# ecmwf-ifs/dwarf-p-cloudsc2-tl-ad

Hardware: AMD Instinct MI355X
Metric: CLOUDSC2 NL columns/sec (fp64, NLEV=137) (higher is better)
Workload: dtype f64

## Files before the change

### dwarf_p_cloudsc2_tl_ad_amd/csrc/cloudsc2_alloc.hip

```cpp

#include <array>
#include "cloudsc2_host.hpp"

using namespace cloudsc2;

namespace {

struct DevAlloc {
  size_t bytes = 0;
  size_t chunk = 0;
  std::vector<hipMemGenericAllocationHandle_t> handles;
};
size_t env_gib(const char* name, size_t dflt) {
  const char* e = getenv(name);
  return (e && atoll(e) > 0) ? (size_t)atoll(e) : dflt;
}
std::mutex g_alloc_mutex;
std::vector<std::pair<void*, DevAlloc>> g_allocs;

size_t search_budget(size_t bytes, size_t free_b) {
  double share = bytes > (env_gib("CLOUDSC2_PLACE_WHOLE_MAX_GB", 12) << 30) ? 0.85 : 0.6;
  if (const char* e = getenv("CLOUDSC2_PLACE_MAX_SHARE")) { const double v = atof(e); if (v > 0.0 && v <= 1.0) share = v; }
  size_t budget = (size_t)(share * (double)free_b);
  const size_t cap = env_gib("CLOUDSC2_PLACE_MAX_GB", 0) << 30;
// ... 243 lines not shown
    int ndev = 0;
    if (lws && hipGetDeviceCount(&ndev) == hipSuccess && ndev > 0) return atoi(lws) > ndev;
    return false;
  }();
  return shared;
}

int device_malloc_impl(void** out, size_t bytes, const ProbeFn* custom, PlacePolicy policy) {
  if (!out) return fail(CLOUDSC2_EINVAL, "cloudsc2_device_malloc: NULL result pointer");
  *out = nullptr;
  if (bytes == 0) return 0;
  std::lock_guard<std::mutex> place_lock(g_place_mutex);
  static const bool allow_custom = !(getenv("CLOUDSC2_PLACE_PROBE") && strcmp(getenv("CLOUDSC2_PLACE_PROBE"), "kernel") != 0);
  struct Scope { Scope(const ProbeFn* f) { g_custom_probe = f; } ~Scope() { g_custom_probe = nullptr; } } scope(allow_custom ? custom : nullptr);
  if (int rc = require_device()) return rc;
  (void)device_prepare();
  static const bool place_env_off = getenv("CLOUDSC2_PLACE") && atoi(getenv("CLOUDSC2_PLACE")) == 0;
  static const bool place_env_on = getenv("CLOUDSC2_PLACE") && atoi(getenv("CLOUDSC2_PLACE")) != 0;
  const bool place = policy == kPlaceSearch ? !place_env_off : (policy == kPlaceOnRequest ? place_env_on : false);
  static const char* mode = getenv("CLOUDSC2_PLACE_MODE");
  const bool chunks = mode && !strcmp(mode, "chunks");
  if (place && chunks && bytes >= (256u << 20)) {
    PlaceStats stc;
    return device_malloc_chunks(out, bytes, stc);
  }
  size_t ncand = 1, budget = 0;
  if (place && bytes >= (256u << 20) && !device_is_shared()) {
    const char* ec = getenv("CLOUDSC2_PLACE_CANDIDATES");
    const size_t span = env_gib("CLOUDSC2_PLACE_SPAN_GB", 96) << 30;
    const size_t want = (ec && atoi(ec) > 0) ? (size_t)atoi(ec) : std::min<size_t>(64, std::max<size_t>(12, (span + bytes - 1) / bytes));
    size_t free_b = 0, total_b = 0;
    HIP_TRY(hipMemGetInfo(&free_b, &total_b));
    budget = search_budget(bytes, free_b);
    ncand = std::max<size_t>(1, std::min(want, budget / bytes));
  }
  std::vector<void*> cand;
  auto grow = [&](size_t n) {
    for (size_t k = 0; k < n; ++k) {
      void* p = nullptr;
      if (hipMalloc(&p, bytes) != hipSuccess) { (void)hipGetLastError(); break; }
      cand.push_back(p);
    }
  };
  grow(ncand);
  if (cand.empty()) {
    (void)hipDeviceSynchronize();
    grow(1);
  }
  if (cand.empty()) { g_err = "cloudsc2_device_malloc: hipMalloc: out of memory"; return (int)hipErrorOutOfMemory; }
  size_t best = 0;
  PlaceStats st;
  if (cand.size() > 1) {
    static const char* pk = getenv("CLOUDSC2_PLACE_PROBE");
    const bool generic = !g_custom_probe;
    const bool use_write = generic && (!pk || strcmp(pk, "mixed") != 0), use_mixed = generic && (!pk || strcmp(pk, "write") != 0);
    std::vector<double> msw, msm;
    hipError_t e = hipSuccess;
    auto probe_from = [&](size_t first) {
      const size_t n = cand.size() - first;
      auto base = [&](size_t k) { return cand[first + k]; };
      std::vector<double> m, w;
      if (!generic) {
        for (size_t k = first; k < cand.size() && e == hipSuccess; ++k) e = hipMemsetAsync(cand[k], 0, bytes, nullptr);
        if (e == hipSuccess) e = probe_all(n, bytes, kProbeCustom, base, m);
      }
      if (use_mixed) e = probe_all(n, bytes, kProbeMixed, base, m);
      if (use_write && e == hipSuccess) e = probe_all(n, bytes, kProbeWrite, base, w);
      msm.insert(msm.end(), m.begin(), m.end());
      msw.insert(msw.end(), w.begin(), w.end());
    };
    probe_from(0);
    if (e == hipSuccess) {
      const std::vector<double>& v = msm.empty() ? msw : msm;
      const double lo = *std::min_element(v.begin(), v.end()), hi = *std::max_element(v.begin(), v.end());
      size_t free_b = 0, total_b = 0;
      if (hi < 1.04 * lo && hipMemGetInfo(&free_b, &total_b) == hipSuccess) {
        const size_t first = cand.size();
        const size_t held = first * bytes, left = budget > held ? budget - held : 0;
        grow(std::min(first, std::min((size_t)(0.7 * (double)free_b), left) / bytes));
        if (cand.size() > first) probe_from(first);
      }
    }
    if (e != hipSuccess) {
      for (auto p : cand) (void)hipFree(p);
      g_err = std::string("cloudsc2_device_malloc: placement probe: ") + hipGetErrorString(e);
      (void)hipGetLastError();
      return (int)e;
    }
    std::vector<double> score(cand.size(), 0.0);
    for (auto* v : {&msw, &msm})
      if (!v->empty()) {
        const double lo = *std::min_element(v->begin(), v->end());
        const double weight = (v == &msw && !msm.empty()) ? 0.2 : 1.0;
        for (size_t k = 0; k < cand.size(); ++k) score[k] += weight * (*v)[k] / lo;
      }
    for (size_t k = 0; k < cand.size(); ++k)
      if (score[k] < score[best]) best = k;
    if (getenv("CLOUDSC2_PLACE_VERBOSE")) {
      fprintf(stderr, "cloudsc2_device_malloc: %zu bytes, %zu candidates, probe ms %s/write:", bytes, cand.size(), generic ? "mixed" : "of the caller's sweep");
      for (size_t k = 0; k < cand.size(); ++k)
        fprintf(stderr, " %s%.4f/%.4f", k == best ? "*" : "", msm.empty() ? 0.0 : msm[k], msw.empty() ? 0.0 : msw[k]);
      fprintf(stderr, "\n");
    }
    std::vector<double> s = msm.empty() ? msw : msm;
    st.best_ms = s[best];
    std::sort(s.begin(), s.end());
    st.median_ms = s[s.size() / 2]; st.worst_ms = s.back();
    for (size_t k = 0; k < cand.size(); ++k)
      if (k != best) (void)hipFree(cand[k]);
    if (getenv("CLOUDSC2_PLACE_VERBOSE")) {
      std::vector<double> one(1, 0.0);
      if (!generic) (void)probe_all(1, bytes, kProbeCustom, [&](size_t) { return cand[best]; }, one);
      double m = 0.0, w = 0.0;
      (void)cloudsc2_device_probe(cand[best], bytes, kProbeMixed, 3, &m);
      (void)cloudsc2_device_probe(cand[best], bytes, kProbeWrite, 3, &w);
      fprintf(stderr, "cloudsc2_device_malloc: the chosen candidate after freeing the others: caller's sweep %.4f mixed %.4f write %.4f ms\n", one[0], m, w);
    }
  }
  st.candidates = (int)cand.size();
  (cand.size() > 1 ? g_searches : g_plain_allocs).fetch_add(1);
  if (getenv("CLOUDSC2_PLACE_VERBOSE") && cand.size() == 1)
    fprintf(stderr, "cloudsc2_device_malloc: %zu bytes, 1 candidate (plain hipMalloc%s)\n", bytes,
            policy == kPlaceSearch ? "" : policy == kPlaceOnRequest ? "; host-array driver workspace: searched only with CLOUDSC2_PLACE=1" : "; staging");
  DevAlloc a;
  a.bytes = bytes;
  std::lock_guard<std::mutex> lock(g_alloc_mutex);
  g_allocs.emplace_back(cand[best], a);
  g_last_place = st;
  *out = cand[best];
  return 0;
}

int device_free_impl(void* p) {
  if (!p) return 0;
  DevAlloc a;
  {
    std::lock_guard<std::mutex> lock(g_alloc_mutex);
    auto it = std::find_if(g_allocs.begin(), g_allocs.end(), [&](const std::pair<void*, DevAlloc>& x) { return x.first == p; });
    if (it == g_allocs.end()) return fail(CLOUDSC2_EINVAL, "cloudsc2_device_free: not a pointer returned by cloudsc2_device_malloc");
    a = it->second;
    g_allocs.erase(it);
  }
  if (a.chunk) {
    HIP_TRY(hipDeviceSynchronize());
    for (size_t k = 0; k < a.handles.size(); ++k) (void)hipMemUnmap((char*)p + k * a.chunk, a.chunk);
    for (auto x : a.handles) (void)hipMemRelease(x);
    (void)hipMemAddressFree(p, a.bytes);
    return 0;
  }
  HIP_TRY(hipFree(p));
  return 0;
}

}

extern "C" {
int cloudsc2_device_malloc(void** ptr, size_t bytes) { return device_malloc_impl(ptr, bytes); }
int cloudsc2_device_free(void* ptr) { return device_free_impl(ptr); }
int cloudsc2_device_probe(void* ptr, size_t bytes, int kind, int rounds, double* ms) {
  if (!ptr || !ms || rounds < 1 || rounds > 64 || (kind != 0 && kind != 1)) return fail(CLOUDSC2_EINVAL, "cloudsc2_device_probe: bad argument");
  if (int rc = require_device()) return rc;
  const long long nblocks = kind == 0 ? (long long)(bytes / (size_t)kProbeBlockBytes) : (long long)(bytes / (size_t)((kMixIn + kMixOut) * kMixBlockElems * 8));
  if (nblocks < 1 || nblocks > 0x7fffffffLL) return fail(CLOUDSC2_EINVAL, "cloudsc2_device_probe: buffer too small or too large");
  hipEvent_t ea = nullptr, eb = nullptr;
  hipError_t e = hipEventCreate(&ea);
  if (e == hipSuccess) e = hipEventCreate(&eb);
  std::vector<float> t;
  for (int r = 0; r <= rounds && e == hipSuccess; ++r) {
    (void)hipEventRecord(ea, nullptr);
    launch_probe(ptr, bytes, kind);
    (void)hipEventRecord(eb, nullptr);
    e = hipEventSynchronize(eb);
    float f = 0;
    if (e == hipSuccess) e = hipEventElapsedTime(&f, ea, eb);
    if (r > 0) t.push_back(f);
  }
  if (ea) (void)hipEventDestroy(ea);
  if (eb) (void)hipEventDestroy(eb);
  if (e != hipSuccess) { g_err = std::string("cloudsc2_device_probe: ") + hipGetErrorString(e); (void)hipGetLastError(); return (int)e; }
  std::sort(t.begin(), t.end());
  *ms = t[t.size() / 2];
  return 0;
}
void cloudsc2_device_malloc_counts(long long* searched, long long* plain) {
  if (searched) *searched = g_searches.load();
  if (plain) *plain = g_plain_allocs.load();
}
void cloudsc2_device_malloc_info(int* candidates, double* best_ms, double* median_ms, double* worst_ms) {
  std::lock_guard<std::mutex> lock(g_alloc_mutex);
  if (candidates) *candidates = g_last_place.candidates;
  if (best_ms) *best_ms = g_last_place.best_ms;
  if (median_ms) *median_ms = g_last_place.median_ms;
  if (worst_ms) *worst_ms = g_last_place.worst_ms;
}
}
```

### dwarf_p_cloudsc2_tl_ad_amd/csrc/cloudsc2_driver.hip

```cpp

#include <thread>
#include "cloudsc2_host.hpp"

using namespace cloudsc2;

namespace {


__global__ void __launch_bounds__(256)
scale_planes_kernel(real_t* dst, long long dst_stride, const real_t* src, long long src_stride, long long plane, long long nblocks,
                    real_t factor) {
  long long i = (long long)blockIdx.x * blockDim.x + threadIdx.x;
  if (i >= plane * nblocks) return;
  long long ibl = i / plane, r = i - ibl * plane;
  dst[ibl * dst_stride + r] = src[ibl * src_stride + r] * factor;
}

__global__ void __launch_bounds__(256)
reblock_kernel(const real_t* __restrict__ src, int np_src, long long stride_src, real_t* __restrict__ dst, int np_dst,
               long long stride_dst, long long nrows, long long ncopy, long long nzero) {
  const long long total = nrows * nzero;
  for (long long e = (long long)blockIdx.x * blockDim.x + threadIdx.x; e < total; e += (long long)gridDim.x * blockDim.x) {
    const long long row = e / nzero, g = e - row * nzero;
    const long long bd = g / np_dst, jd = g - bd * np_dst;
    real_t v = 0;
    if (g < ncopy) {
      const long long bs = g / np_src, js = g - bs * np_src;
      v = src[bs * stride_src + row * np_src + js];
    }
    dst[bd * stride_dst + row * np_dst + jd] = v;
  }
}

constexpr size_t kAlignReals = 256 / sizeof(real_t);
size_t r32(size_t n) { return (n + kAlignReals - 1) & ~(kAlignReals - 1); }
constexpr size_t kF64 = sizeof(double) / sizeof(real_t);

struct Arena {
  real_t* base = nullptr;
  size_t cap = 0, used = 0;
  int device = -1;

  int reserve(size_t nreals, const ProbeFn* probe = nullptr, PlacePolicy policy = kPlaceSearch) {
    int dev = 0;
    HIP_TRY(hipGetDevice(&dev));
    if (base && (cap < nreals || dev != device)) { (void)device_free_impl(base); base = nullptr; cap = 0; }
    if (!base) {
      int rc = device_malloc_impl((void**)&base, nreals * sizeof(real_t), probe, policy);
      if (rc) { base = nullptr; return rc; }
      cap = nreals;
      device = dev;
    }
    used = 0;
    return 0;
  }
  real_t* take(size_t n) {
    n = r32(n);
    real_t* p = base + used;
    used += n;
    return p;
  }
  double* take_f64(size_t n) { return (double*)take(n * (sizeof(double) / sizeof(real_t))); }
  void release() {
    if (base) (void)device_free_impl(base);
    base = nullptr; cap = 0; used = 0;
  }
};
Arena g_arena;
std::mutex g_arena_mutex;

struct DevState {
  real_t *pt, *pq, *b_cml, *b_loc, *pap, *paph, *plu, *plude, *pmfu, *pmfd, *pa, *pclv, *psupsat, *pcovptot;
  real_t *pfplsl, *pfplsn, *pfhpsl, *pfhpsn, *qsat;
  long long S, H;
  long long nblocks;
};

size_t state_out_reals(long long ncols_pad, int nlev) {
  size_t s = (size_t)ncols_pad * nlev, h = (size_t)ncols_pad * (nlev + 1);
  return 3 * r32(s) + 4 * r32(h) + r32(8 * s);
}
size_t state_in_reals(long long ncols_pad, int nlev) {
  size_t s = (size_t)ncols_pad * nlev, h = (size_t)ncols_pad * (nlev + 1);
  return 8 * r32(s) + r32(h) + r32(8 * s) + r32(5 * s);
}
size_t state_reals(long long ncols_pad, int nlev) { return state_in_reals(ncols_pad, nlev) + state_out_reals(ncols_pad, nlev); }

void state_take(Arena& a, DevState& d, long long ncols_pad, int nproma, int nlev) {
  Arena& ain = a;
  Arena& aout = a;
  size_t s = (size_t)ncols_pad * nlev, h = (size_t)ncols_pad * (nlev + 1);
  d.S = (long long)nproma * nlev;
  d.H = (long long)nproma * (nlev + 1);
  d.nblocks = ncols_pad / nproma;
  d.pt = ain.take(s); d.pq = ain.take(s); d.pap = ain.take(s); d.plu = ain.take(s); d.plude = ain.take(s);
  d.pmfu = ain.take(s); d.pmfd = ain.take(s); d.psupsat = ain.take(s);
  d.paph = ain.take(h); d.b_cml = ain.take(8 * s); d.pclv = ain.take(5 * s);
  d.pa = aout.take(s); d.pcovptot = aout.take(s); d.qsat = aout.take(s);
  d.pfplsl = aout.take(h); d.pfplsn = aout.take(h); d.pfhpsl = aout.take(h); d.pfhpsn = aout.take(h);
  d.b_loc = aout.take(8 * s);
}

struct HostState {
  const real_t *pt, *pq, *b_cml; real_t* b_loc;
  const real_t *pap, *paph, *plu, *plude, *pmfu, *pmfd; real_t* pa; const real_t *pclv, *psupsat;
  real_t *pcovptot, *pfplsl, *pfplsn, *pfhpsl, *pfhpsn;
};

int copy_planes(real_t* dst, const real_t* src, long long plane_off, long long plane, long long block_stride, long long nblocks,
                hipMemcpyKind kind, hipStream_t st) {
  if (nblocks <= 0) return 0;
  HIP_TRY(hipMemcpy2DAsync(dst + plane_off, block_stride * sizeof(real_t), src + plane_off, block_stride * sizeof(real_t),
                           plane * sizeof(real_t), (size_t)nblocks, kind, st));
  return 0;
}

int upload(const HostState& h, const DevState& d, long long ncols_pad, int nlev, hipStream_t st) {
  size_t s = (size_t)ncols_pad * nlev * sizeof(real_t), hh = (size_t)ncols_pad * (nlev + 1) * sizeof(real_t);
  const long long P = d.S;
  HIP_TRY(hipMemcpyAsync(d.pt, h.pt, s, hipMemcpyHostToDevice, st));
  HIP_TRY(hipMemcpyAsync(d.pq, h.pq, s, hipMemcpyHostToDevice, st));
  HIP_TRY(hipMemcpyAsync(d.pap, h.pap, s, hipMemcpyHostToDevice, st));
  HIP_TRY(hipMemcpyAsync(d.paph, h.paph, hh, hipMemcpyHostToDevice, st));
  HIP_TRY(hipMemcpyAsync(d.plu, h.plu, s, hipMemcpyHostToDevice, st));
  HIP_TRY(hipMemcpyAsync(d.plude, h.plude, s, hipMemcpyHostToDevice, st));
  HIP_TRY(hipMemcpyAsync(d.pmfu, h.pmfu, s, hipMemcpyHostToDevice, st));
  HIP_TRY(hipMemcpyAsync(d.pmfd, h.pmfd, s, hipMemcpyHostToDevice, st));
  HIP_TRY(hipMemcpyAsync(d.psupsat, h.psupsat, s, hipMemcpyHostToDevice, st));
  int rc;
  for (int p : {0, 2, 3, 4})
    if ((rc = copy_planes(d.b_cml, h.b_cml, p * P, P, 8 * P, d.nblocks, hipMemcpyHostToDevice, st))) return rc;
  for (int p : {0, 1})
    if ((rc = copy_planes(d.pclv, h.pclv, p * P, P, 5 * P, d.nblocks, hipMemcpyHostToDevice, st))) return rc;
  return 0;
}

int download_active2(real_t* hdst, long long hstride, const real_t* dsrc, long long dstride, long long nlevx, int nproma,
                     long long ngptot, hipStream_t st) {
  const long long nfull = ngptot / nproma, icend = ngptot - nfull * nproma;
  const long long plane = (long long)nproma * nlevx;
  if (nfull > 0) {
    if (hstride == plane && dstride == plane) {
      HIP_TRY(hipMemcpyAsync(hdst, dsrc, (size_t)nfull * plane * sizeof(real_t), hipMemcpyDeviceToHost, st));
    } else {
      HIP_TRY(hipMemcpy2DAsync(hdst, hstride * sizeof(real_t), dsrc, dstride * sizeof(real_t), plane * sizeof(real_t), (size_t)nfull,
                               hipMemcpyDeviceToHost, st));
    }
  }
  if (icend > 0) {
    HIP_TRY(hipMemcpy2DAsync(hdst + nfull * hstride, (size_t)nproma * sizeof(real_t), dsrc + nfull * dstride, (size_t)nproma * sizeof(real_t),
                             (size_t)icend * sizeof(real_t), (size_t)nlevx, hipMemcpyDeviceToHost, st));
  }
  return 0;
}
int download_active(real_t* hdst, const real_t* dsrc, long long plane_off, long long nlevx, long long block_stride, int nproma,
                    long long ngptot, hipStream_t st) {
  return download_active2(hdst + plane_off, block_stride, dsrc + plane_off, block_stride, nlevx, nproma, ngptot, st);
}

int download(const HostState& h, const DevState& d, long long ncols_pad, int nlev, hipStream_t st, int nproma, long long ngptot) {
  const long long P = d.S, PH = d.H;
  int rc;
  for (int p : {0, 2, 3, 4})
    if ((rc = download_active(h.b_loc, d.b_loc, p * P, nlev, 8 * P, nproma, ngptot, st))) return rc;
  if ((rc = copy_planes(h.b_loc, d.b_loc, 7 * P, P, 8 * P, d.nblocks, hipMemcpyDeviceToHost, st))) return rc;
  if ((rc = download_active(h.pa, d.pa, 0, nlev, P, nproma, ngptot, st))) return rc;
  HIP_TRY(hipMemcpyAsync(h.pcovptot, d.pcovptot, (size_t)ncols_pad * nlev * sizeof(real_t), hipMemcpyDeviceToHost, st));
  if ((rc = download_active(h.pfplsl, d.pfplsl, 0, nlev + 1, PH, nproma, ngptot, st))) return rc;
  if ((rc = download_active(h.pfplsn, d.pfplsn, 0, nlev + 1, PH, nproma, ngptot, st))) return rc;
  if ((rc = download_active(h.pfhpsl, d.pfhpsl, 0, nlev + 1, PH, nproma, ngptot, st))) return rc;
  if ((rc = download_active(h.pfhpsn, d.pfhpsn, 0, nlev + 1, PH, nproma, ngptot, st))) return rc;
  return 0;
}

cloudsc2_field fld(real_t* p, long long stride) { cloudsc2_field f; f.ptr = p; f.block_stride = stride; return f; }

void traj_blocks(const DevState& d, int nproma, int nlev, bool with_qsat, cloudsc2_inputs& in, cloudsc2_outputs& out) {
  const long long S = d.S, H = d.H, P = (long long)nproma * nlev;
  in.paph = fld(d.paph, H); in.pap = fld(d.pap, S); in.q = fld(d.pq, S);
  in.qsat = fld(with_qsat ? d.qsat : nullptr, S); in.t = fld(d.pt, S);
  in.l = fld(d.pclv + 0 * P, 5 * S); in.i = fld(d.pclv + 1 * P, 5 * S);
  in.lude = fld(d.plude, S); in.lu = fld(d.plu, S); in.mfu = fld(d.pmfu, S); in.mfd = fld(d.pmfd, S);
  in.gtent = fld(d.b_cml + 0 * P, 8 * S); in.gtenq = fld(d.b_cml + 2 * P, 8 * S);
  in.gtenl = fld(d.b_cml + 3 * P, 8 * S); in.gteni = fld(d.b_cml + 4 * P, 8 * S);
  in.supsat = fld(d.psupsat, S);
  out.tent = fld(d.b_loc + 0 * P, 8 * S); out.tenq = fld(d.b_loc + 2 * P, 8 * S);
  out.tenl = fld(d.b_loc + 3 * P, 8 * S); out.teni = fld(d.b_loc + 4 * P, 8 * S);
  out.clc = fld(d.pa, S); out.covptot = fld(d.pcovptot, S);
  out.fplsl = fld(d.pfplsl, H); out.fplsn = fld(d.pfplsn, H); out.fhpsl = fld(d.pfhpsl, H); out.fhpsn = fld(d.pfhpsn, H);
}

ProbeFn state_probe(int nproma, int nlev, int ngptot) {
  return [=](void* base, size_t bytes) {
    cloudsc2_params prm;
    cloudsc2_params_default(&prm);
    prm.nlev = nlev;
    prm.math_mode = 1;
    for (int k = 0; k < nlev && k < CLOUDSC2_MAX_NLEV; ++k) prm.ceta[k] = (k + 0.5) / nlev;
    Geom g;
    if (check_geom(&prm, nproma, nlev, ngptot, g)) return;
    if (state_reals(g.ncols_pad, nlev) * sizeof(real_t) > bytes) return;
    Arena view;
    view.base = (real_t*)base;
    view.cap = bytes / sizeof(real_t);
    DevState d;
    state_take(view, d, g.ncols_pad, nproma, nlev);
    cloudsc2_inputs in; cloudsc2_outputs out;
    traj_blocks(d, nproma, nlev, false, in, out);
    const cloudsc2_field zero = fld(d.b_loc + 7LL * nproma * nlev, 8 * d.S);
    (void)cloudsc2_nl_launch(&prm, 3600.0, nproma, nlev, ngptot, &in, &out, zero, 0.0, nullptr);
  };
}

const ProbeFn* judge_for(const ProbeFn& nl_probe, size_t total, size_t state) {
  return (total > state && (total - state) * sizeof(real_t) >= (256u << 20)) ? nullptr : &nl_probe;
}

struct FlatIn { cloudsc2_inputs in; };
void flat_in_take(Arena& a, long long ncols_pad, int nproma, int nlev, cloudsc2_inputs& in) {
  size_t s = (size_t)ncols_pad * nlev, h = (size_t)ncols_pad * (nlev + 1);
  const long long S = (long long)nproma * nlev, H = (long long)nproma * (nlev + 1);
  in.paph = fld(a.take(h), H);
  cloudsc2_field* f[15] = {&in.pap, &in.q, &in.qsat, &in.t, &in.l, &in.i, &in.lude, &in.lu, &in.mfu, &in.mfd,
                           &in.gtent, &in.gtenq, &in.gtenl, &in.gteni, &in.supsat};
  for (auto p : f) *p = fld(a.take(s), S);
}
void flat_out_take(Arena& a, long long ncols_pad, int nproma, int nlev, cloudsc2_outputs& out) {
  size_t s = (size_t)ncols_pad * nlev, h = (size_t)ncols_pad * (nlev + 1);
  const long long S = (long long)nproma * nlev, H = (long long)nproma * (nlev + 1);
  cloudsc2_field* f[6] = {&out.tent, &out.tenq, &out.tenl, &out.teni, &out.clc, &out.covptot};
  for (auto p : f) *p = fld(a.take(s), S);
  cloudsc2_field* g[4] = {&out.fplsl, &out.fplsn, &out.fhpsl, &out.fhpsn};
  for (auto p : g) *p = fld(a.take(h), H);
}
constexpr int kPairPlanes = 26;
bool pair_blocked(int nproma) { return nproma < 64; }
size_t pair_reals(long long ncols_pad, int nlev) { return r32((size_t)kPairPlanes * (size_t)ncols_pad * (nlev + 1)); }
void pair_take(Arena& a, long long ncols_pad, int nproma, int nlev, cloudsc2_inputs& in, cloudsc2_outputs& out) {
  if (!pair_blocked(nproma)) {
    flat_in_take(a, ncols_pad, nproma, nlev, in);
    flat_out_take(a, ncols_pad, nproma, nlev, out);
    return;
  }
  const long long plane = (long long)nproma * (nlev + 1), stride = kPairPlanes * plane;
  real_t* base = a.take((size_t)kPairPlanes * (size_t)ncols_pad * (nlev + 1));
  cloudsc2_field* fi[16] = {&in.paph, &in.pap, &in.q, &in.qsat, &in.t, &in.l, &in.i, &in.lude, &in.lu, &in.mfu, &in.mfd,
                            &in.gtent, &in.gtenq, &in.gtenl, &in.gteni, &in.supsat};
  cloudsc2_field* fo[10] = {&out.tent, &out.tenq, &out.tenl, &out.teni, &out.clc, &out.fplsl, &out.fplsn, &out.fhpsl, &out.fhpsn,
                            &out.covptot};
  for (int k = 0; k < 16; ++k) *fi[k] = fld(base + k * plane, stride);
  for (int k = 0; k < 10; ++k) *fo[k] = fld(base + (16 + k) * plane, stride);
}

size_t flat_in_reals(long long ncols_pad, int nlev) { return 15 * r32((size_t)ncols_pad * nlev) + r32((size_t)ncols_pad * (nlev + 1)); }
size_t flat_out_reals(long long ncols_pad, int nlev) { return 6 * r32((size_t)ncols_pad * nlev) + 4 * r32((size_t)ncols_pad * (nlev + 1)); }

struct Timer {
  hipEvent_t a = nullptr, b = nullptr;
  Timer() = default;
  Timer(const Timer&) = delete;
  Timer& operator=(const Timer&) = delete;
  ~Timer() {
    if (a) (void)hipEventDestroy(a);
    if (b) (void)hipEventDestroy(b);
  }
  int start(hipStream_t st) {
    HIP_TRY(hipEventCreate(&a));
    HIP_TRY(hipEventCreate(&b));
    HIP_TRY(hipEventRecord(a, st));
    return 0;
  }
  int stop(hipStream_t st, double* ms) {
    HIP_TRY(hipEventRecord(b, st));
    HIP_TRY(hipEventSynchronize(b));
    float f = 0;
    HIP_TRY(hipEventElapsedTime(&f, a, b));
    if (ms) *ms = f;
    return 0;
  }
};

struct SlabResources {
  hipStream_t s_up = nullptr, s_k = nullptr;
  std::vector<hipEvent_t> ev;
  SlabResources() = default;
  SlabResources(const SlabResources&) = delete;
  SlabResources& operator=(const SlabResources&) = delete;
  ~SlabResources() {
    for (auto e : ev) if (e) (void)hipEventDestroy(e);
    if (s_up) (void)hipStreamDestroy(s_up);
    if (s_k) (void)hipStreamDestroy(s_k);
  }
  int create(size_t nevents) {
    HIP_TRY(hipStreamCreateWithFlags(&s_up, hipStreamNonBlocking));
    HIP_TRY(hipStreamCreateWithFlags(&s_k, hipStreamNonBlocking));
    ev.assign(nevents, nullptr);
    for (auto& e : ev) HIP_TRY(hipEventCreate(&e));
    return 0;
  }
};

HostState host_view(const HostState& h, long long b0, const DevState& d) {
  const long long S = d.S, H = d.H;
  HostState v = h;
  v.pt += b0 * S; v.pq += b0 * S; v.b_cml += b0 * 8 * S; v.b_loc += b0 * 8 * S; v.pap += b0 * S; v.paph += b0 * H;
  v.plu += b0 * S; v.plude += b0 * S; v.pmfu += b0 * S; v.pmfd += b0 * S; v.pa += b0 * S; v.pclv += b0 * 5 * S;
  v.psupsat += b0 * S; v.pcovptot += b0 * S; v.pfplsl += b0 * H; v.pfplsn += b0 * H; v.pfhpsl += b0 * H; v.pfhpsn += b0 * H;
  return v;
}
DevState dev_view(const DevState& d, long long b0, long long nb) {
  const long long S = d.S, H = d.H;
  DevState v = d;
  v.pt += b0 * S; v.pq += b0 * S; v.b_cml += b0 * 8 * S; v.b_loc += b0 * 8 * S; v.pap += b0 * S; v.paph += b0 * H;
  v.plu += b0 * S; v.plude += b0 * S; v.pmfu += b0 * S; v.pmfd += b0 * S; v.pa += b0 * S; v.pclv += b0 * 5 * S;
  v.psupsat += b0 * S; v.pcovptot += b0 * S; v.pfplsl += b0 * H; v.pfplsn += b0 * H; v.pfhpsl += b0 * H; v.pfhpsn += b0 * H;
  v.qsat += b0 * S;
  v.nblocks = nb;
  return v;
}

int upload_slab_sync(const HostState& h, const DevState& d, long long ncols, int nlev, hipStream_t st) {
  int rc = upload(h, d, ncols, nlev, st);
  if (rc) return rc;
  HIP_TRY(hipStreamSynchronize(st));
  return 0;
}

int nl_run_slabs(const cloudsc2_params* prm, double ptsphy, int nproma, int nlev, int ngptot, const Geom& g, const HostState& h,
                 const DevState& d, double* kernel_ms) {
  const long long nb = d.nblocks;
  const long long slab_blocks = std::max<long long>(1, 16384 / nproma);
  const long long nslabs = (nb + slab_blocks - 1) / slab_blocks;
  int device = 0;
  HIP_TRY(hipGetDevice(&device));
  SlabResources res;
  {
    const int rc_res = res.create((size_t)(2 * nslabs));
    if (rc_res) return rc_res;
  }
  const hipStream_t s_up = res.s_up, s_k = res.s_k;
  const std::vector<hipEvent_t>& ev = res.ev;

  std::atomic<long long> uploaded{0};
  std::atomic<int> up_rc{0};
  std::string up_err;
  auto slab_cols = [&](long long i, long long& b0, long long& nbs, long long& active) {
    b0 = i * slab_blocks;
    nbs = std::min(slab_blocks, nb - b0);
    active = std::min<long long>(nbs * nproma, (long long)ngptot - b0 * nproma);
  };
  std::thread uploader([&] {
    if (hipSetDevice(device) != hipSuccess) { up_rc = CLOUDSC2_EINVAL; up_err = "hipSetDevice failed in the upload thread"; return; }
    for (long long i = 0; i < nslabs && up_rc == 0; ++i) {
      long long b0, nbs, active;
      slab_cols(i, b0, nbs, active);
      int rc = upload_slab_sync(host_view(h, b0, d), dev_view(d, b0, nbs), nbs * nproma, nlev, s_up);
      if (rc) { up_err = g_err; up_rc = rc; return; }
      uploaded.store(i + 1, std::memory_order_release);
    }
  });

  int rc = 0;
  for (long long i = 0; i < nslabs && rc == 0; ++i) {
    while (uploaded.load(std::memory_order_acquire) <= i && up_rc == 0) std::this_thread::yield();
    if (up_rc != 0) break;
    long long b0, nbs, active;
    slab_cols(i, b0, nbs, active);
    const DevState dv = dev_view(d, b0, nbs);
    cloudsc2_inputs in; cloudsc2_outputs out;
    traj_blocks(dv, nproma, nlev, false, in, out);
    if (hipEventRecord(ev[2 * i], s_k) != hipSuccess) { rc = fail(CLOUDSC2_EINVAL, "hipEventRecord failed"); break; }
    rc = cloudsc2_nl_launch(prm, ptsphy, nproma, nlev, (int)active, &in, &out, fld(dv.b_loc + 7LL * nproma * nlev, 8 * dv.S), 0.0, s_k);
    if (rc) break;
    if (hipEventRecord(ev[2 * i + 1], s_k) != hipSuccess) { rc = fail(CLOUDSC2_EINVAL, "hipEventRecord failed"); break; }
    rc = download(host_view(h, b0, d), dv, nbs * nproma, nlev, s_k, nproma, active);
  }
  uploader.join();
  if (rc == 0 && up_rc != 0) rc = fail(up_rc, up_err.c_str());
  const hipError_t e_sync = hipStreamSynchronize(s_k);
  if (rc == 0 && e_sync != hipSuccess) rc = fail(CLOUDSC2_EINVAL, hipGetErrorString(e_sync));
  if (rc == 0 && kernel_ms) {
    double total = 0.0;
    for (long long i = 0; i < nslabs; ++i) {
      float f = 0.f;
      if (hipEventElapsedTime(&f, ev[2 * i], ev[2 * i + 1]) == hipSuccess) total += f;
    }
    *kernel_ms = total;
  }
  (void)g;
  return rc;
}

}

extern "C" {

void cloudsc2_release_workspace(void) {
  std::lock_guard<std::mutex> lock(g_arena_mutex);
  g_arena.release();
}

int cloudsc2_nl_run(const cloudsc2_params* prm, int nproma, int nlev, int ngptot, double ptsphy, const cloudsc2_real* pt,
                    const cloudsc2_real* pq, const cloudsc2_real* b_cml, cloudsc2_real* b_loc, const cloudsc2_real* pap, const cloudsc2_real* paph,
                    const cloudsc2_real* plu, const cloudsc2_real* plude, const cloudsc2_real* pmfu, const cloudsc2_real* pmfd, cloudsc2_real* pa,
                    const cloudsc2_real* pclv, const cloudsc2_real* psupsat, cloudsc2_real* pcovptot, cloudsc2_real* pfplsl, cloudsc2_real* pfplsn,
                    cloudsc2_real* pfhpsl, cloudsc2_real* pfhpsn, double* kernel_ms) {
  Geom g;
  int rc = check_geom(prm, nproma, nlev, ngptot, g);
  if (rc) return rc;
  std::lock_guard<std::mutex> lock(g_arena_mutex);
  const ProbeFn probe = state_probe(nproma, nlev, ngptot);
  if ((rc = g_arena.reserve(state_reals(g.ncols_pad, nlev), &probe, kPlaceOnRequest))) return rc;
  DevState d;
  state_take(g_arena, d, g.ncols_pad, nproma, nlev);
  HostState h = {pt, pq, b_cml, b_loc, pap, paph, plu, plude, pmfu, pmfd, pa, pclv, psupsat, pcovptot, pfplsl, pfplsn, pfhpsl, pfhpsn};
  return nl_run_slabs(prm, ptsphy, nproma, nlev, ngptot, g, h, d, kernel_ms);
}

}
namespace {

size_t taylor_nsums(int ngptot, int nproma_stat) { return (size_t)(((long long)ngptot + nproma_stat - 1) / nproma_stat) * 10 * 2 * 10; }
size_t taylor_ws_reals(long long ncols_pad, int nproma, int nlev, int ngptot, int nproma_stat) {
  (void)nproma;
  const size_t nsums = taylor_nsums(ngptot, nproma_stat);
  return std::max(flat_in_reals(ncols_pad, nlev) + flat_out_reals(ncols_pad, nlev), pair_reals(ncols_pad, nlev)) +
         r32((size_t)(10 * kTaylorLambdas + 10) * (size_t)ncols_pad * kF64) + r32(nsums * kF64);
}
size_t adjoint_ws_reals(long long ncols_pad, int nlev) {
  const size_t ncol = (size_t)ncols_pad;
  return std::max(flat_in_reals(ncols_pad, nlev) + flat_out_reals(ncols_pad, nlev), pair_reals(ncols_pad, nlev)) + r32(ncol * nlev) +
         r32(3 * ncol * kF64) + r32(32 * kF64);
}

int taylor_compute(const cloudsc2_params* prm_in, const Geom& g, int nproma, int nlev, int ngptot, double ptsphy, const DevState& d,
                   Arena& ws, double znormg[10], double* kernel_ms, hipStream_t st, int nproma_stat) {
  const long long nblocks_stat = ((long long)ngptot + nproma_stat - 1) / nproma_stat;
  const size_t nsums = taylor_nsums(ngptot, nproma_stat);
  cloudsc2_inputs inc;
  cloudsc2_outputs tlo;
  pair_take(ws, g.ncols_pad, nproma, nlev, inc, tlo);
  (void)inc;
  double* colsum = ws.take_f64((size_t)(10 * kTaylorLambdas + 10) * (size_t)g.ncols_pad);
  double* sums = ws.take_f64(nsums);
  int rc;
  cloudsc2_inputs in; cloudsc2_outputs out;
  traj_blocks(d, nproma, nlev, true, in, out);
  cloudsc2_params prm_call = *prm_in;
  if (prm_call.math_mode == 0) prm_call.math_mode = 2;
  const cloudsc2_params* prm = &prm_call;
  Timer tm;
  if ((rc = tm.start(st))) return rc;
  HIP_TRY(hipMemsetAsync(d.pcovptot, 0, (size_t)g.ncols_pad * nlev * sizeof(real_t), st));
  {
    const long long plane = (long long)nproma * nlev, nblocks = g.ncols_pad / nproma, n = plane * nblocks;
    hipLaunchKernelGGL(scale_planes_kernel, dim3((unsigned)((n + 255) / 256)), dim3(256), 0, st, d.b_loc + 7 * plane, 8 * d.S,
                       (const real_t*)(d.b_loc + 7 * plane), 8 * d.S, plane, nblocks, RC(0.0));
  }
  if ((rc = cloudsc2_satur_launch(prm, nproma, nlev, ngptot, in.pap, in.t, in.qsat, st))) return rc;
  if ((rc = cloudsc2_tl_launch_self(prm, ptsphy, nproma, nlev, ngptot, &in, &out, 0.01, &tlo, nullptr, st))) return rc;
  if ((rc = cloudsc2_taylor_sweep_launch(prm, ptsphy, nproma, nlev, ngptot, nproma_stat, &in, &out, &tlo, colsum, sums, st))) return rc;
  if ((rc = tm.stop(st, kernel_ms))) return rc;
  std::vector<double> hs(nsums);
  HIP_TRY(hipMemcpyAsync(hs.data(), sums, nsums * sizeof(double), hipMemcpyDeviceToHost, st));
  HIP_TRY(hipStreamSynchronize(st));

  const double eps = sizeof(real_t) == 4 ? 1.1920928955078125e-07 : 2.220446049250313e-16;
  for (int il = 0; il < 10; ++il) {
    double zg = 0.0;
    for (long long b = 0; b < nblocks_stat; ++b) {
      double znorm = 0.0, zcount = 0.0;
      for (int f = 0; f < 10; ++f) {
        const double* p = &hs[((size_t)il * nblocks_stat + b) * 20 + f * 2];
        if (fabs(p[1]) > eps) {
          zcount += 1.0;
          znorm += fabs(p[0] / p[1]);
        }
      }
      if (znorm == 0.0 || zcount == 0.0) return fail(CLOUDSC2_ETLWRONG, "TL is totally wrong !!! (a block has no active statistics)");
      zg = fmax(zg, znorm / zcount);
    }
    znormg[il] = zg;
  }
  return 0;
}

int adjoint_compute(const cloudsc2_params* prm, const Geom& g, int nproma, int nlev, int ngptot, double ptsphy, const DevState& d,
                    Arena& ws, double* znormg, double* kernel_ms, hipStream_t st) {
  const long long nblocks = g.ncols_pad / nproma;
  const size_t ncol = (size_t)g.ncols_pad;
  cloudsc2_inputs x;
  cloudsc2_outputs y;
  pair_take(ws, g.ncols_pad, nproma, nlev, x, y);
  real_t* scratch = ws.take(ncol * nlev);
  double* norms = ws.take_f64(3 * ncol);
  double* gmax = ws.take_f64(32);
  int rc;
  cloudsc2_inputs in; cloudsc2_outputs out;
  traj_blocks(d, nproma, nlev, true, in, out);
  HIP_TRY(hipMemsetAsync(gmax, 0, sizeof(double), st));
  HIP_TRY(hipMemsetAsync(norms, 0, 3 * ncol * sizeof(double), st));
  Timer tm;
  if ((rc = tm.start(st))) return rc;
  HIP_TRY(hipMemsetAsync(d.pcovptot, 0, ncol * nlev * sizeof(real_t), st));
  {
    long long plane = (long long)nproma * nlev;
    long long n = plane * nblocks;
    hipLaunchKernelGGL(scale_planes_kernel, dim3((unsigned)((n + 255) / 256)), dim3(256), 0, st, d.b_loc + 7 * plane, 8 * d.S,
                       (const real_t*)(d.b_loc + 7 * plane), 8 * d.S, plane, nblocks, RC(0.0));
  }
  if ((rc = cloudsc2_satur_launch(prm, nproma, nlev, ngptot, in.pap, in.t, in.qsat, st))) return rc;
  const bool evap = prm->levapls2 || prm->ldrain1d;
  const char* full = getenv("CLOUDSC2_AD_SYMMETRY_FULL");
  if (evap || (full && atoi(full) != 0)) {
    if ((rc = cloudsc2_tl_launch_self(prm, ptsphy, nproma, nlev, ngptot, &in, &out, 0.0, &y, nullptr, st))) return rc;
    if ((rc = cloudsc2_adjoint_norms_launch(nproma, nlev, ngptot, nullptr, nullptr, &y, nullptr, norms, gmax, st))) return rc;
    if ((rc = cloudsc2_ad_launch_assign(prm, ptsphy, nproma, nlev, ngptot, &in, &out, &x, &y, scratch, st))) return rc;
    cloudsc2_field qf = in.qsat;
    if ((rc = cloudsc2_adjoint_norms_launch(nproma, nlev, ngptot, &in, &qf, nullptr, &x, norms, gmax, st))) return rc;
  } else {
    if ((rc = cloudsc2_tl_launch_self(prm, ptsphy, nproma, nlev, ngptot, &in, &out, 0.0, &y, norms, st))) return rc;
    if ((rc = cloudsc2_ad_launch_reverse_norms(prm, ptsphy, nproma, nlev, ngptot, &in, &out, &x, &y, norms, gmax, st))) return rc;
  }
  if ((rc = tm.stop(st, kernel_ms))) return rc;
  double hmax = 0.0;
  HIP_TRY(hipMemcpyAsync(&hmax, gmax, sizeof(double), hipMemcpyDeviceToHost, st));
  HIP_TRY(hipStreamSynchronize(st));
  *znormg = hmax;
  return 0;
}

}

struct cloudsc2_state {
  int nproma = 0, nproma_user = 0, nlev = 0, ngptot = 0, device = 0;
  long long ncols_pad_user = 0;
  Geom g;
  Arena arena, ws, tmp;
  DevState d;
};

namespace {
struct FieldSpec { int nlevx_extra; int ndim; };
int state_field(const cloudsc2_state* s, int field, cloudsc2_field* f, int* nlevx) {
  const DevState& d = s->d;
  const long long S = d.S, H = d.H, P = (long long)s->nproma * s->nlev;
  real_t* full[] = {d.pt, d.pq, d.pap, nullptr, d.plu, d.plude, d.pmfu, d.pmfd, d.pa, d.psupsat, d.pcovptot};
  *nlevx = s->nlev;
  if (field >= CLOUDSC2_F_PT && field <= CLOUDSC2_F_PCOVPTOT && field != CLOUDSC2_F_PAPH) { *f = fld(full[field], S); return 0; }
  switch (field) {
    case CLOUDSC2_F_PAPH: *f = fld(d.paph, H); *nlevx = s->nlev + 1; return 0;
// ... 297 lines not shown
```

### dwarf_p_cloudsc2_tl_ad_amd/csrc/cloudsc2_host.hpp

```cpp
#pragma once
#include <hip/hip_runtime.h>
#include <math.h>
#include <stdio.h>
#include <stdlib.h>
#include <string.h>

#include <algorithm>
#include <atomic>
#include <functional>
#include <initializer_list>
#include <mutex>
#include <string>
#include <utility>
#include <vector>

#include "../../include/cloudsc2_hip.h"
#include "cloudsc2_sweep_kernels.hpp"

namespace cloudsc2 {

extern thread_local std::string g_err;
int fail(int code, const char* msg);

#define HIP_TRY(expr)                                                                     \
  do {                                                                                    \
    hipError_t e_ = (expr);                                                               \
    if (e_ != hipSuccess) {                                                               \
      g_err = std::string(#expr) + ": " + hipGetErrorString(e_);                          \
      return (int)e_;                                                                     \
    }                                                                                     \
  } while (0)

bool device_ok();
int no_device();
inline int require_device() { return device_ok() ? 0 : no_device(); }

bool precise_of(const cloudsc2_params* prm);
int check_geom(const cloudsc2_params* prm, int nproma, int nlev, int ngptot, Geom& g);
int resolve_in(const cloudsc2_inputs& in, bool need_qsat, Strides& s, InPtrs& p);
int resolve_out(const cloudsc2_outputs& out, bool all_required, Strides& s, OutPtrs& p);
int get_tables(const cloudsc2_params& p, const LevelTab** dev, int* kb0, int* kb1);
int validate_launch_impl(const cloudsc2_real* table, int klon, int period, long long start, int nlevx, int ndim, int nproma,
                         long long ngptot, cloudsc2_field field, double* workspace, double* stats, void* stream, long long ncols_minmax);

inline unsigned grid_for(long long ncols, int block) { return (unsigned)((ncols + block - 1) / block); }

template <class Args>
int launch_variant(KernelFn<Args> fn, const Args& args, long long ncols, hipStream_t st) {
  if (!fn) return fail(CLOUDSC2_EINVAL, "kernel variant not built");
  Args a = args;
  void* argv[] = {&a};
  HIP_TRY(hipLaunchKernel((const void*)fn, dim3(grid_for(ncols, kBlock)), dim3(kBlock), argv, 0, st));
  return 0;
}

void schedule(Geom& g, const void* fair, bool nap, const void* pace);
int device_prepare();

bool device_is_shared();
using ProbeFn = std::function<void(void* base, size_t bytes)>;
enum PlacePolicy { kPlaceSearch = 0, kPlaceOnRequest = 1, kPlacePlain = 2 };
int device_malloc_impl(void** out, size_t bytes, const ProbeFn* custom = nullptr, PlacePolicy policy = kPlaceSearch);
int device_free_impl(void* p);

}
```

Measured before the change: 207.9 million.

## Stage slab transfers through pinned host ring with multithreaded gather and scatter

Replaces the per-slab synchronous upload thread with a double-buffered pinned host ring. Worker threads gather host planes into the pinned slots and scatter results back out, while uploads, kernels and downloads run on three separate streams linked by events. Stream, event and buffer resources are kept in a persistent global object instead of being recreated on every call. The aim is to get DMA from pinned memory and to overlap H2D, compute and D2H across slabs, at the cost of extra host memcpy passes and added threading complexity.

```diff
diff --git a/dwarf_p_cloudsc2_tl_ad_amd/csrc/cloudsc2_alloc.hip b/dwarf_p_cloudsc2_tl_ad_amd/csrc/cloudsc2_alloc.hip
--- a/dwarf_p_cloudsc2_tl_ad_amd/csrc/cloudsc2_alloc.hip
+++ b/dwarf_p_cloudsc2_tl_ad_amd/csrc/cloudsc2_alloc.hip
@@ -419,6 +419,21 @@
   return 0;
 }
 
+int host_pinned_malloc_impl(void** out, size_t bytes) {
+  if (!out) return fail(CLOUDSC2_EINVAL, "NULL result pointer");
+  *out = nullptr;
+  if (bytes == 0) return 0;
+  if (int rc = require_device()) return rc;
+  HIP_TRY(hipHostMalloc(out, bytes, hipHostMallocDefault));
+  return 0;
+}
+
+int host_pinned_free_impl(void* p) {
+  if (!p) return 0;
+  HIP_TRY(hipHostFree(p));
+  return 0;
+}
+
 }
 
 extern "C" {
diff --git a/dwarf_p_cloudsc2_tl_ad_amd/csrc/cloudsc2_driver.hip b/dwarf_p_cloudsc2_tl_ad_amd/csrc/cloudsc2_driver.hip
--- a/dwarf_p_cloudsc2_tl_ad_amd/csrc/cloudsc2_driver.hip
+++ b/dwarf_p_cloudsc2_tl_ad_amd/csrc/cloudsc2_driver.hip
@@ -1,6 +1,8 @@
 
+#include <memory>
 #include <thread>
 #include "cloudsc2_host.hpp"
+#include "cloudsc2_staging.hpp"
 
 using namespace cloudsc2;
 
@@ -280,25 +282,79 @@
   }
 };
 
-struct SlabResources {
-  hipStream_t s_up = nullptr, s_k = nullptr;
+constexpr int kSlots = 2;
+constexpr int kUpPlanes = 14, kDownPlanes = 7, kDownHalf = 4;
+
+struct HostPipe {
+  int device = -1;
+  hipStream_t s_up = nullptr, s_k = nullptr, s_down = nullptr;
+  hipEvent_t up_done[kSlots] = {}, down_done[kSlots] = {};
   std::vector<hipEvent_t> ev;
-  SlabResources() = default;
-  SlabResources(const SlabResources&) = delete;
-  SlabResources& operator=(const SlabResources&) = delete;
-  ~SlabResources() {
+  real_t* ring = nullptr;
+  size_t up_reals = 0, down_reals = 0;
+  std::unique_ptr<staging::Workers> gatherers, scatterers;
+
+  real_t* up_slot(int s) const { return ring + (size_t)s * up_reals; }
+  real_t* down_slot(int s) const { return ring + (size_t)kSlots * up_reals + (size_t)s * down_reals; }
+
+  int prepare(size_t up, size_t down, size_t nevents) {
+    int dev = 0;
+    HIP_TRY(hipGetDevice(&dev));
+    if (device >= 0 && dev != device) release();
+    hipStreamCaptureMode mode = hipStreamCaptureModeRelaxed;
+    const bool exchanged = hipThreadExchangeStreamCaptureMode(&mode) == hipSuccess;
+    const int rc = make(dev, up, down, nevents);
+    if (exchanged) (void)hipThreadExchangeStreamCaptureMode(&mode);
+    return rc;
+  }
+  int make(int dev, size_t up, size_t down, size_t nevents) {
+    device = dev;
+    for (hipStream_t* s : {&s_up, &s_k, &s_down})
+      if (!*s) HIP_TRY(hipStreamCreateWithFlags(s, hipStreamNonBlocking));
+    for (int k = 0; k < kSlots; ++k) {
+      if (!up_done[k]) HIP_TRY(hipEventCreateWithFlags(&up_done[k], hipEventDisableTiming | hipEventBlockingSync));
+      if (!down_done[k]) HIP_TRY(hipEventCreateWithFlags(&down_done[k], hipEventDisableTiming | hipEventBlockingSync));
+    }
+    while (ev.size() < nevents) {
+      hipEvent_t e = nullptr;
+      HIP_TRY(hipEventCreate(&e));
+      ev.push_back(e);
+    }
+    if (!ring || up > up_reals || down > down_reals) {
+      if (ring) (void)host_pinned_free_impl(ring);
+      ring = nullptr;
+      up_reals = std::max(up, up_reals);
+      down_reals = std::max(down, down_reals);
+      const int rc = host_pinned_malloc_impl((void**)&ring, (size_t)kSlots * (up_reals + down_reals) * sizeof(real_t));
+      if (rc) { ring = nullptr; up_reals = down_reals = 0; return rc; }
+    }
+    if (!gatherers) {
+      const int nt = (int)std::min(4u, std::max(1u, std::thread::hardware_concurrency() / 2));
+      gatherers.reset(new staging::Workers(nt));
+      scatterers.reset(new staging::Workers(nt));
+    }
+    return 0;
+  }
+  void release() {
+    gatherers.reset();
+    scatterers.reset();
+    if (ring) (void)host_pinned_free_impl(ring);
+    ring = nullptr; up_reals = down_reals = 0;
     for (auto e : ev) if (e) (void)hipEventDestroy(e);
-    if (s_up) (void)hipStreamDestroy(s_up);
-    if (s_k) (void)hipStreamDestroy(s_k);
-  }
-  int create(size_t nevents) {
-    HIP_TRY(hipStreamCreateWithFlags(&s_up, hipStreamNonBlocking));
-    HIP_TRY(hipStreamCreateWithFlags(&s_k, hipStreamNonBlocking));
-    ev.assign(nevents, nullptr);
-    for (auto& e : ev) HIP_TRY(hipEventCreate(&e));
-    return 0;
+    ev.clear();
+    for (int k = 0; k < kSlots; ++k) {
+      if (up_done[k]) (void)hipEventDestroy(up_done[k]);
+      if (down_done[k]) (void)hipEventDestroy(down_done[k]);
+      up_done[k] = down_done[k] = nullptr;
+    }
+    for (hipStream_t* s : {&s_up, &s_k, &s_down}) {
+      if (*s) (void)hipStreamDestroy(*s);
+      *s = nullptr;
+    }
+    device = -1;
   }
 };
+HostPipe* g_pipe = nullptr;
 
 HostState host_view(const HostState& h, long long b0, const DevState& d) {
   const long long S = d.S, H = d.H;
@@ -319,71 +375,124 @@
   return v;
 }
 
-int upload_slab_sync(const HostState& h, const DevState& d, long long ncols, int nlev, hipStream_t st) {
-  int rc = upload(h, d, ncols, nlev, st);
-  if (rc) return rc;
-  HIP_TRY(hipStreamSynchronize(st));
-  return 0;
+using Pass = std::vector<staging::PlaneCopy<real_t>>;
+constexpr int kCmlUp[4] = {0, 2, 3, 4}, kClvUp[2] = {0, 1}, kLocDown[5] = {0, 2, 3, 4, 7};
+
+Pass gather_pass(const HostState& h, const DevState& d, real_t* slot, long long cap, int nproma, int nlev) {
+  const long long P = d.S, PH = d.H, nbs = d.nblocks;
+  Pass pass;
+  const real_t* full[8] = {h.pt, h.pq, h.pap, h.plu, h.plude, h.pmfu, h.pmfd, h.psupsat};
+  for (int k = 0; k < 8; ++k) pass.push_back({slot + k * cap * P, P, full[k], P, nlev, nproma, nbs, nproma});
+  for (int k = 0; k < 4; ++k) pass.push_back({slot + (8 + k) * cap * P, P, h.b_cml + kCmlUp[k] * P, 8 * P, nlev, nproma, nbs, nproma});
+  for (int k = 0; k < 2; ++k) pass.push_back({slot + (12 + k) * cap * P, P, h.pclv + kClvUp[k] * P, 5 * P, nlev, nproma, nbs, nproma});
+  pass.push_back({slot + kUpPlanes * cap * P, PH, h.paph, PH, nlev + 1, nproma, nbs, nproma});
+  return pass;
+}
+int enqueue_upload(const DevState& d, const real_t* slot, long long cap, hipStream_t st) {
+  const long long P = d.S, PH = d.H, nbs = d.nblocks;
+  const size_t sz = sizeof(real_t);
+  real_t* full[8] = {d.pt, d.pq, d.pap, d.plu, d.plude, d.pmfu, d.pmfd, d.psupsat};
+  for (int k = 0; k < 8; ++k) HIP_TRY(hipMemcpyAsync(full[k], slot + k * cap * P, (size_t)(nbs * P) * sz, hipMemcpyHostToDevice, st));
+  for (int k = 0; k < 4; ++k)
+    HIP_TRY(hipMemcpy2DAsync(d.b_cml + kCmlUp[k] * P, 8 * P * sz, slot + (8 + k) * cap * P, P * sz, P * sz, (size_t)nbs, hipMemcpyHostToDevice, st));
+  for (int k = 0; k < 2; ++k)
+    HIP_TRY(hipMemcpy2DAsync(d.pclv + kClvUp[k] * P, 5 * P * sz, slot + (12 + k) * cap * P, P * sz, P * sz, (size_t)nbs, hipMemcpyHostToDevice, st));
+  HIP_TRY(hipMemcpyAsync(d.paph, slot + kUpPlanes * cap * P, (size_t)(nbs * PH) * sz, hipMemcpyHostToDevice, st));
+  return 0;
+}
+int enqueue_download(const DevState& d, real_t* slot, long long cap, hipStream_t st) {
+  const long long P = d.S, PH = d.H, nbs = d.nblocks;
+  const size_t sz = sizeof(real_t);
+  for (int k = 0; k < 5; ++k)
+    HIP_TRY(hipMemcpy2DAsync(slot + k * cap * P, P * sz, d.b_loc + kLocDown[k] * P, 8 * P * sz, P * sz, (size_t)nbs, hipMemcpyDeviceToHost, st));
+  HIP_TRY(hipMemcpyAsync(slot + 5 * cap * P, d.pa, (size_t)(nbs * P) * sz, hipMemcpyDeviceToHost, st));
+  HIP_TRY(hipMemcpyAsync(slot + 6 * cap * P, d.pcovptot, (size_t)(nbs * P) * sz, hipMemcpyDeviceToHost, st));
+  const real_t* half[4] = {d.pfplsl, d.pfplsn, d.pfhpsl, d.pfhpsn};
+  real_t* base = slot + kDownPlanes * cap * P;
+  for (int k = 0; k < 4; ++k) HIP_TRY(hipMemcpyAsync(base + k * cap * PH, half[k], (size_t)(nbs * PH) * sz, hipMemcpyDeviceToHost, st));
+  return 0;
+}
+Pass scatter_pass(const HostState& h, const DevState& d, const real_t* slot, long long cap, int nproma, int nlev, long long active) {
+  const long long P = d.S, PH = d.H, nbs = d.nblocks;
+  const long long last = active - (nbs - 1) * nproma;
+  Pass pass;
+  for (int k = 0; k < 5; ++k)
+    pass.push_back({h.b_loc + kLocDown[k] * P, 8 * P, slot + k * cap * P, P, nlev, nproma, nbs, kLocDown[k] == 7 ? nproma : last});
+  pass.push_back({h.pa, P, slot + 5 * cap * P, P, nlev, nproma, nbs, last});
+  pass.push_back({h.pcovptot, P, slot + 6 * cap * P, P, nlev, nproma, nbs, nproma});
+  real_t* half[4] = {h.pfplsl, h.pfplsn, h.pfhpsl, h.pfhpsn};
+  const real_t* base = slot + kDownPlanes * cap * P;
+  for (int k = 0; k < 4; ++k) pass.push_back({half[k], PH, base + k * cap * PH, PH, nlev + 1, nproma, nbs, last});
+  return pass;
 }
 
 int nl_run_slabs(const cloudsc2_params* prm, double ptsphy, int nproma, int nlev, int ngptot, const Geom& g, const HostState& h,
                  const DevState& d, double* kernel_ms) {
   const long long nb = d.nblocks;
-  const long long slab_blocks = std::max<long long>(1, 16384 / nproma);
-  const long long nslabs = (nb + slab_blocks - 1) / slab_blocks;
-  int device = 0;
-  HIP_TRY(hipGetDevice(&device));
-  SlabResources res;
-  {
-    const int rc_res = res.create((size_t)(2 * nslabs));
-    if (rc_res) return rc_res;
-  }
-  const hipStream_t s_up = res.s_up, s_k = res.s_k;
-  const std::vector<hipEvent_t>& ev = res.ev;
-
-  std::atomic<long long> uploaded{0};
-  std::atomic<int> up_rc{0};
-  std::string up_err;
-  auto slab_cols = [&](long long i, long long& b0, long long& nbs, long long& active) {
-    b0 = i * slab_blocks;
-    nbs = std::min(slab_blocks, nb - b0);
-    active = std::min<long long>(nbs * nproma, (long long)ngptot - b0 * nproma);
+  long long slab_cols = 16384;
+  if (const char* e = getenv("CLOUDSC2_SLAB_COLUMNS")) {
+    if (atoll(e) > 0) slab_cols = atoll(e);
+  }
+  const long long cap = std::min(nb, std::max<long long>(1, slab_cols / nproma));
+  const long long nslabs = (nb + cap - 1) / cap;
+  if (!g_pipe) g_pipe = new HostPipe;
+  HostPipe& pipe = *g_pipe;
+  int rc = pipe.prepare(r32((size_t)cap * (kUpPlanes * d.S + d.H)), r32((size_t)cap * (kDownPlanes * d.S + kDownHalf * d.H)), (size_t)(2 * nslabs));
+  if (rc) return rc;
+  const int device = pipe.device;
+  std::vector<long long> scattered((size_t)nslabs, -1);
+
+  auto check = [&](hipError_t e, const char* what) {
+    if (e == hipSuccess) return 0;
+    return fail(CLOUDSC2_EINVAL, (std::string(what) + ": " + hipGetErrorString(e)).c_str());
   };
-  std::thread uploader([&] {
-    if (hipSetDevice(device) != hipSuccess) { up_rc = CLOUDSC2_EINVAL; up_err = "hipSetDevice failed in the upload thread"; return; }
-    for (long long i = 0; i < nslabs && up_rc == 0; ++i) {
-      long long b0, nbs, active;
-      slab_cols(i, b0, nbs, active);
-      int rc = upload_slab_sync(host_view(h, b0, d), dev_view(d, b0, nbs), nbs * nproma, nlev, s_up);
-      if (rc) { up_err = g_err; up_rc = rc; return; }
-      uploaded.store(i + 1, std::memory_order_release);
-    }
-  });
-
-  int rc = 0;
   for (long long i = 0; i < nslabs && rc == 0; ++i) {
-    while (uploaded.load(std::memory_order_acquire) <= i && up_rc == 0) std::this_thread::yield();
-    if (up_rc != 0) break;
-    long long b0, nbs, active;
-    slab_cols(i, b0, nbs, active);
+    const int slot = (int)(i % kSlots);
+    const long long b0 = i * cap, nbs = std::min(cap, nb - b0);
+    const long long active = std::min<long long>(nbs * nproma, (long long)ngptot - b0 * nproma);
+    const HostState hv = host_view(h, b0, d);
     const DevState dv = dev_view(d, b0, nbs);
+    if (i >= kSlots && (rc = check(hipEventSynchronize(pipe.up_done[slot]), "hipEventSynchronize (upload)"))) break;
+    {
+      const Pass pass = gather_pass(hv, dv, pipe.up_slot(slot), cap, nproma, nlev);
+      pipe.gatherers->wait(pipe.gatherers->post([pass](int t, int nt, std::string&) { staging::copy_share(pass, t, nt); return 0; }));
+    }
+    if ((rc = enqueue_upload(dv, pipe.up_slot(slot), cap, pipe.s_up))) break;
+    if ((rc = check(hipEventRecord(pipe.up_done[slot], pipe.s_up), "hipEventRecord"))) break;
+    if ((rc = check(hipStreamWaitEvent(pipe.s_k, pipe.up_done[slot], 0), "hipStreamWaitEvent"))) break;
     cloudsc2_inputs in; cloudsc2_outputs out;
     traj_blocks(dv, nproma, nlev, false, in, out);
-    if (hipEventRecord(ev[2 * i], s_k) != hipSuccess) { rc = fail(CLOUDSC2_EINVAL, "hipEventRecord failed"); break; }
-    rc = cloudsc2_nl_launch(prm, ptsphy, nproma, nlev, (int)active, &in, &out, fld(dv.b_loc + 7LL * nproma * nlev, 8 * dv.S), 0.0, s_k);
-    if (rc) break;
-    if (hipEventRecord(ev[2 * i + 1], s_k) != hipSuccess) { rc = fail(CLOUDSC2_EINVAL, "hipEventRecord failed"); break; }
-    rc = download(host_view(h, b0, d), dv, nbs * nproma, nlev, s_k, nproma, active);
-  }
-  uploader.join();
-  if (rc == 0 && up_rc != 0) rc = fail(up_rc, up_err.c_str());
-  const hipError_t e_sync = hipStreamSynchronize(s_k);
-  if (rc == 0 && e_sync != hipSuccess) rc = fail(CLOUDSC2_EINVAL, hipGetErrorString(e_sync));
+    if ((rc = check(hipEventRecord(pipe.ev[2 * i], pipe.s_k), "hipEventRecord"))) break;
+    if ((rc = cloudsc2_nl_launch(prm, ptsphy, nproma, nlev, (int)active, &in, &out, fld(dv.b_loc + 7LL * nproma * nlev, 8 * dv.S), 0.0, pipe.s_k))) break;
+    if ((rc = check(hipEventRecord(pipe.ev[2 * i + 1], pipe.s_k), "hipEventRecord"))) break;
+    if (i >= kSlots) pipe.scatterers->wait(scattered[(size_t)(i - kSlots)]);
+    if ((rc = check(hipStreamWaitEvent(pipe.s_down, pipe.ev[2 * i + 1], 0), "hipStreamWaitEvent"))) break;
+    if ((rc = enqueue_download(dv, pipe.down_slot(slot), cap, pipe.s_down))) break;
+    const hipEvent_t arrived = pipe.down_done[slot];
+    if ((rc = check(hipEventRecord(arrived, pipe.s_down), "hipEventRecord"))) break;
+    const Pass pass = scatter_pass(hv, dv, pipe.down_slot(slot), cap, nproma, nlev, active);
+    scattered[(size_t)i] = pipe.scatterers->post([pass, arrived, device](int t, int nt, std::string& text) {
+      hipError_t e = hipSetDevice(device);
+      if (e == hipSuccess) e = hipEventSynchronize(arrived);
+      if (e != hipSuccess) { text = std::string("download: ") + hipGetErrorString(e); return (int)CLOUDSC2_EINVAL; }
+      staging::copy_share(pass, t, nt);
+      return 0;
+    });
+  }
+  pipe.gatherers->wait_all();
+  pipe.scatterers->wait_all();
+  std::string text;
+  const int rc_scatter = pipe.scatterers->take_error(text);
+  if (rc == 0 && rc_scatter != 0) rc = fail(rc_scatter, text.c_str());
+  for (hipStream_t s : {pipe.s_up, pipe.s_k, pipe.s_down}) {
+    const hipError_t e_sync = hipStreamSynchronize(s);
+    if (rc == 0 && e_sync != hipSuccess) rc = fail(CLOUDSC2_EINVAL, hipGetErrorString(e_sync));
+  }
   if (rc == 0 && kernel_ms) {
     double total = 0.0;
     for (long long i = 0; i < nslabs; ++i) {
       float f = 0.f;
-      if (hipEventElapsedTime(&f, ev[2 * i], ev[2 * i + 1]) == hipSuccess) total += f;
+      if (hipEventElapsedTime(&f, pipe.ev[2 * i], pipe.ev[2 * i + 1]) == hipSuccess) total += f;
     }
     *kernel_ms = total;
   }
@@ -397,6 +506,11 @@
 
 void cloudsc2_release_workspace(void) {
   std::lock_guard<std::mutex> lock(g_arena_mutex);
+  if (g_pipe) {
+    g_pipe->release();
+    delete g_pipe;
+    g_pipe = nullptr;
+  }
   g_arena.release();
 }
 
diff --git a/dwarf_p_cloudsc2_tl_ad_amd/csrc/cloudsc2_host.hpp b/dwarf_p_cloudsc2_tl_ad_amd/csrc/cloudsc2_host.hpp
--- a/dwarf_p_cloudsc2_tl_ad_amd/csrc/cloudsc2_host.hpp
+++ b/dwarf_p_cloudsc2_tl_ad_amd/csrc/cloudsc2_host.hpp
@@ -62,5 +62,7 @@
 enum PlacePolicy { kPlaceSearch = 0, kPlaceOnRequest = 1, kPlacePlain = 2 };
 int device_malloc_impl(void** out, size_t bytes, const ProbeFn* custom = nullptr, PlacePolicy policy = kPlaceSearch);
 int device_free_impl(void* p);
+int host_pinned_malloc_impl(void** out, size_t bytes);
+int host_pinned_free_impl(void* p);
 
 }
diff --git a/dwarf_p_cloudsc2_tl_ad_amd/csrc/cloudsc2_staging.hpp b/dwarf_p_cloudsc2_tl_ad_amd/csrc/cloudsc2_staging.hpp
--- /dev/null
+++ b/dwarf_p_cloudsc2_tl_ad_amd/csrc/cloudsc2_staging.hpp
@@ -0,0 +1,133 @@
+#pragma once
+#include <string.h>
+
+#include <condition_variable>
+#include <deque>
+#include <functional>
+#include <mutex>
+#include <string>
+#include <thread>
+#include <vector>
+
+namespace cloudsc2 {
+namespace staging {
+
+template <class T>
+struct PlaneCopy {
+  T* dst;
+  long long dst_stride;
+  const T* src;
+  long long src_stride;
+  long long nlevx;
+  int nproma;
+  long long nblocks;
+  long long active_last;
+};
+
+template <class T>
+void copy_share(const PlaneCopy<T>& c, int t, int nt) {
+  const long long b0 = c.nblocks * t / nt, b1 = c.nblocks * (t + 1) / nt;
+  if (b1 <= b0) return;
+  const long long plane = (long long)c.nproma * c.nlevx;
+  const bool ragged = c.active_last < c.nproma;
+  const long long whole_end = (ragged && b1 == c.nblocks) ? b1 - 1 : b1;
+  if (whole_end > b0) {
+    if (c.dst_stride == plane && c.src_stride == plane) {
+      memcpy(c.dst + b0 * plane, c.src + b0 * plane, (size_t)((whole_end - b0) * plane) * sizeof(T));
+    } else {
+      for (long long b = b0; b < whole_end; ++b) memcpy(c.dst + b * c.dst_stride, c.src + b * c.src_stride, (size_t)plane * sizeof(T));
+    }
+  }
+  if (whole_end < b1 && c.active_last > 0) {
+    T* d = c.dst + whole_end * c.dst_stride;
+    const T* s = c.src + whole_end * c.src_stride;
+    for (long long jk = 0; jk < c.nlevx; ++jk) memcpy(d + jk * c.nproma, s + jk * c.nproma, (size_t)c.active_last * sizeof(T));
+  }
+}
+
+template <class T>
+void copy_share(const std::vector<PlaneCopy<T>>& pass, int t, int nt) {
+  for (const auto& c : pass) copy_share(c, t, nt);
+}
+
+class Workers {
+ public:
+  using Task = std::function<int(int t, int nt, std::string& text)>;
+  explicit Workers(int nt) {
+    for (int t = 0; t < nt; ++t) th_.emplace_back([this, t, nt] { loop(t, nt); });
+  }
+  Workers(const Workers&) = delete;
+  Workers& operator=(const Workers&) = delete;
+  ~Workers() {
+    {
+      std::lock_guard<std::mutex> lk(m_);
+      stop_ = true;
+    }
+    work_.notify_all();
+    for (auto& t : th_) t.join();
+  }
+  int size() const { return (int)th_.size(); }
+  long long post(Task task) {
+    long long n;
+    {
+      std::lock_guard<std::mutex> lk(m_);
+      q_.push_back({std::move(task), 0});
+      n = first_ + (long long)q_.size() - 1;
+    }
+    work_.notify_all();
+    return n;
+  }
+  void wait(long long n) {
+    std::unique_lock<std::mutex> lk(m_);
+    done_.wait(lk, [&] { return n < first_ || q_[(size_t)(n - first_)].finished == (int)th_.size(); });
+    while (!q_.empty() && q_.front().finished == (int)th_.size()) { q_.pop_front(); ++first_; }
+  }
+  void wait_all() {
+    long long last;
+    {
+      std::lock_guard<std::mutex> lk(m_);
+      last = first_ + (long long)q_.size() - 1;
+    }
+    if (last >= 0) wait(last);
+  }
+  int take_error(std::string& text) {
+    std::lock_guard<std::mutex> lk(m_);
+    const int rc = rc_;
+    if (rc) text = text_;
+    rc_ = 0;
+    text_.clear();
+    return rc;
+  }
+
+ private:
+  struct Entry { Task task; int finished; };
+  void loop(int t, int nt) {
+    long long next = 0;
+    std::unique_lock<std::mutex> lk(m_);
+    for (;;) {
+      work_.wait(lk, [&] { return stop_ || next < first_ + (long long)q_.size(); });
+      if (stop_) return;
+      if (next < first_) next = first_;
+      Task& task = q_[(size_t)(next - first_)].task;
+      lk.unlock();
+      std::string text;
+      const int rc = task(t, nt, text);
+      lk.lock();
+      if (rc && !rc_) { rc_ = rc; text_ = text; }
+      ++q_[(size_t)(next - first_)].finished;
+      ++next;
+      done_.notify_all();
+    }
+  }
+  std::mutex m_;
+  std::condition_variable work_, done_;
+  std::deque<Entry> q_;
+  long long first_ = 0;
+  bool stop_ = false;
+  int rc_ = 0;
+  std::string text_;
+  std::vector<std::thread> th_;
+};
+
+}
+}
```

After: 207.4 million. Within noise of the previous version (-0.2%).
